# dharunm236/TempME

Hardware: AMD Instinct MI355X
Metric: explained target-edges/sec (TGN+Enron, n_degree=20) at 1/2/4/8 MI355X (higher is better)
Workload: dtype fp32

## Files before the change

include/tempme.h:

```cpp
#ifndef TEMPME_H_
#define TEMPME_H_

#include <stdint.h>

#ifdef __cplusplus
extern "C" {
#endif

#define TM_OK 0
#define TM_E_EDGE_NOT_IN_LIST (-1)
#define TM_E_SHAPE (-2)
#define TM_E_HIP (-3)
#define TM_E_ARG (-4)
#define TM_E_UNSUPPORTED (-5)

#define TM_SIDE_NONE 0
#define TM_SIDE_SRC 1
#define TM_SIDE_TGT 2
#define TM_SIDE_BGD 3
#define TM_STAGE_STEP2 16
#define TM_STAGE_STEP3 17
#define TM_STAGE_NEG 32
#define TM_STAGE_PERM 48
#define TM_SPLIT_TRAIN 0
#define TM_SPLIT_TEST 1
#define TM_SPLIT_NULL 2

typedef struct tm_graph tm_graph;
typedef struct tm_weights tm_weights;
typedef struct tm_dropin tm_dropin;

typedef struct {
    uint64_t seed;
    uint32_t split;
    uint32_t side;
} tm_rng;

const char *tm_last_error(void);
int tm_version(void);

#define TM_DEBUG_FORCE_UNKEYED 1
#define TM_DEBUG_HOST_BUILD 2
#define TM_DEBUG_GRAPH_TIMING 3
#define TM_DEBUG_WALK_BLOCKS 4
#define TM_DEBUG_N_OPTS 5
int tm_debug_set(int32_t opt, int32_t value);
int tm_set_host_threads(int32_t n);

int tm_graph_build(int32_t n_nodes, const int64_t *in_off, const int32_t *ngh, const int32_t *eid,
                   const double *ts, int device, tm_graph **out);
int tm_graph_build_edges(int32_t n_nodes, int64_t n_edges, const int64_t *src, const int64_t *dst,
                         const int64_t *eidx, const double *ts, int device, tm_graph **out);
int tm_graph_free(tm_graph *g);
int tm_graph_info(const tm_graph *g, int32_t *n_nodes, int64_t *n_entries, int32_t *max_eid);
int tm_graph_export(const tm_graph *g, int64_t *off, int32_t *ngh, int32_t *eid, double *ts, int32_t *dict_val);
int tm_graph_strict_view(const tm_graph *g, tm_graph **out);

int tm_sample_khop(const tm_graph *g, tm_rng rng, int32_t k, int32_t N, int32_t B, const int32_t *root,
                   const double *cut, const int32_t *eidx, const uint32_t *event_ids, int32_t *out_node,
                   int32_t *out_eid, float *out_ts, int32_t *err_flag, void *stream);

int tm_sample_walks(const tm_graph *g, tm_rng rng, int32_t N, int32_t M, int32_t B, const int32_t *root,
                    const int32_t *h1_node, const int32_t *h1_eid, const float *h1_ts, const uint32_t *event_ids,
                    int32_t *out_node6, int32_t *out_eid3, float *out_ts3, int32_t *out_anony3, int32_t *out_cat,
                    void *stream);

int tm_neg_sample(tm_rng rng, const int32_t *list, int64_t n_list, const uint32_t *event_ids, int32_t n, int32_t j,
                  int32_t *out, void *stream);
// ... 353 lines not shown
```

tempme_amd/_lib.py:

```python
import ctypes as C
import os
import types

import torch

_HERE = os.path.dirname(os.path.abspath(__file__))
LIB_PATH = os.environ.get("TEMPME_LIB") or os.path.join(_HERE, "lib", "libtempme_hip.so")

TM_OK = 0
TM_E_EDGE_NOT_IN_LIST = -1
TM_E_SHAPE = -2
TM_E_HIP = -3
TM_E_ARG = -4
TM_E_UNSUPPORTED = -5

SIDE_NONE, SIDE_SRC, SIDE_TGT, SIDE_BGD = 0, 1, 2, 3
SPLIT_TRAIN, SPLIT_TEST, SPLIT_NULL = 0, 1, 2
TM_DEBUG_FORCE_UNKEYED, TM_DEBUG_HOST_BUILD, TM_DEBUG_GRAPH_TIMING, TM_DEBUG_WALK_BLOCKS = 1, 2, 3, 4
N_WEIGHTS = 28

EXPORTS = (
    "tm_last_error", "tm_version", "tm_debug_set", "tm_set_host_threads", "tm_graph_build", "tm_graph_build_edges", "tm_graph_free", "tm_graph_info", "tm_graph_export",
    "tm_graph_strict_view",
    "tm_sample_khop", "tm_sample_walks", "tm_neg_sample", "tm_perm_keys", "tm_motif_hist", "tm_edge_counts",
    "tm_sample_events", "tm_gather_rows", "tm_weights_create", "tm_weights_create_ex", "tm_weights_pack", "tm_weights_variant", "tm_weights_set_node_zero", "tm_weights_version", "tm_weights_free",
    "tm_weight_split3", "tm_weight_gcn_split", "tm_encoder_workspace_bytes",
    "tm_walk_importance", "tm_encoder_pool_workspace_bytes", "tm_encoder_pool_fwd",
    "tm_encoder_pool_train_workspace_bytes", "tm_encoder_pool_train_fwd", "tm_encoder_pool_bwd", "tm_encoder_pool_wgrad",
    "tm_encoder_fwd", "tm_encoder_fwd_tab", "tm_encoder_train_supported", "tm_encoder_train_fwd", "tm_encoder_bwd", "tm_encoder_wgrad", "tm_wgrad",
    "tm_explain_train_fwd", "tm_explain_train_fwd_pad", "tm_explain_train_bwd", "tm_kl_loss", "tm_edge_importance", "tm_edge_gate_table",
    "tm_edge_table_cols", "tm_edge_tables", "tm_edge_feature_table", "tm_edge_importance_tab", "tm_tgn_attn_fwd", "tm_tgn_attn_bwd", "tm_tgn_attn_train_fwd", "tm_tgn_attn_train_bwd", "tm_tgn_attn_train_workspace_bytes", "tm_tgn_attn_train_dtab", "tm_tgn_rows_reduce", "tm_tgat_attn_fwd", "tm_tgat_attn_bwd", "tm_tgat_merge_fwd", "tm_tgat_attn_train_workspace_bytes", "tm_tgat_attn_train_fwd", "tm_tgat_attn_train_bwd", "tm_gm_packed_floats", "tm_gm_pack", "tm_gm_embed", "tm_gm_embed_bwd_ok", "tm_gm_embed_bwd", "tm_gm_packed_a_floats", "tm_gm_pack_a", "tm_gm_fused_ok", "tm_gm_train_ok", "tm_gm_train_workspace_bytes", "tm_gm_train_fwd", "tm_gm_train_bwd", "tm_dropin_create", "tm_dropin_free", "tm_dropin_forward", "tm_dropin_set_stream", "tm_dropin_gate_cache", "tm_dropin_gate_cache_clear", "tm_edge_importance_gf", "tm_edge_importance_gf3", "tm_edge_importance_gf3_bern",
    "tm_mask_least_important", "tm_profile_enable", "tm_profile_sync", "tm_profile_entry",
    "tm_beta_params", "tm_beta_rsample_bwd", "tm_adam_step", "tm_adam_step_gated", "tm_copy_many", "tm_host_register", "tm_host_unregister",
    "tm_stage_cast",
)


class TmRng(C.Structure):
    _fields_ = [("seed", C.c_uint64), ("split", C.c_uint32), ("side", C.c_uint32)]


# ... 296 lines not shown
```

tempme_amd/csrc/encoder.hip:

```cpp
#include <algorithm>
#include <atomic>
#include <cstring>
#include <vector>

#include "encoder_common.h"

namespace tmk {

__device__ __forceinline__ double block_sum(double v, double *red) {
#pragma unroll
    for (int o = 32; o > 0; o >>= 1) v += __shfl_xor(v, o);
    const int wave = threadIdx.x >> 6, nw = blockDim.x >> 6;
    __syncthreads();
    if ((threadIdx.x & 63) == 0) red[wave] = v;
    __syncthreads();
    double s = 0.0;
    for (int k = 0; k < nw; ++k) s += red[k];
    return s;
}

__global__ void __launch_bounds__(1024) std_kernel(int32_t B, int32_t W, const double *__restrict__ cut,
                                                   const float *__restrict__ ts3, float *__restrict__ std_out) {
    __shared__ double red[16];
    const int64_t g = blockIdx.x;
// ... 518 lines not shown
        o[t] = __builtin_amdgcn_mfma_f32_16x16x4f32(w.z, x[q].z, o[t], 0, 0, 0);
        p[t] = __builtin_amdgcn_mfma_f32_16x16x4f32(w.z, y[q].z, p[t], 0, 0, 0);
        o[t] = __builtin_amdgcn_mfma_f32_16x16x4f32(w.w, x[q].w, o[t], 0, 0, 0);
        p[t] = __builtin_amdgcn_mfma_f32_16x16x4f32(w.w, y[q].w, p[t], 0, 0, 0);
        __builtin_amdgcn_sched_barrier(0);
    }
}

template <int NQE>
struct WalkLay {
    static constexpr int EV = FoldLay::SIZE, EVB = EV + 11 * NQE * 256, G1 = EVB + 176, G1B = G1 + 4 * 11 * 256,
                         G2 = G1B + 64, G2B = G2 + 4 * 4 * 256, W1 = G2B + 64, W1B = W1 + 8 * 8 * 256, W2 = W1B + 128,
                         W2B = W2 + 8 * 8 * 256, A1 = W2B + 128, A1B = A1 + 4 * 8 * 256, A2 = A1B + 64,
                         A2B = A2 + 4 * 4 * 256, M1 = A2B + 64, M1B = M1 + 5 * 5 * 256, M2 = M1B + 80,
                         M2B = M2 + 4 * 5 * 256;
};

constexpr int PFP = 4;
constexpr int WALK_WAVES = 2;
constexpr int WALK_WPB = 4;

constexpr int GCN_LDS = 3;
constexpr int GCN_LDS_FRAGS = GCN_LDS * 12;
constexpr int gcn_step(int k, int gl, int ns) {
    const int nstr = ns - gl, m = nstr < gl ? nstr : gl;
    if (k < 2 * m) return (k & 1) ? k / 2 : gl + k / 2;
    return nstr > gl ? gl + k - m : k - m;
}

template <int NTO, int NQ, int NQL, int BASE>
__device__ __forceinline__ void cgemm(__amdgpu_buffer_rsrc_t wr, const floatx4 (&x)[NQ], floatx4 (&o)[NTO]) {
    using O = PairOrder<NTO, NQ>;
    const int vo = lane_id() * 16;
    constexpr int N = NTO * NQ, D = PFP < N ? PFP : N;
    auto off = [](int i) { return BASE / 4 + (O::t(i) * NQL + O::q(i)) * 64; };
    float4 buf[D];
#pragma unroll
    for (int i = 0; i < D; ++i) buf[i] = wload(wr, vo, off(i));
#pragma unroll
    for (int k = 0; k < O::NP * NQ; ++k) {
        const int i = 2 * k, t = O::t(i), q = O::q(i);
        const float4 w0 = buf[i % D];
        if (i + D < N) buf[i % D] = wload(wr, vo, off(i + D));
        const float4 w1 = buf[(i + 1) % D];
        if (i + 1 + D < N) buf[(i + 1) % D] = wload(wr, vo, off(i + 1 + D));
        o[t] = __builtin_amdgcn_mfma_f32_16x16x4f32(w0.x, x[q].x, o[t], 0, 0, 0);
// ... 154 lines not shown
__device__ __forceinline__ floatx4 relu_add4(const floatx4 &a, const float4 &b) {
    return floatx4{relu(a[0] + b.x), relu(a[1] + b.y), relu(a[2] + b.z), relu(a[3] + b.w)};
}

__device__ __forceinline__ floatx4 relu4(const floatx4 &a) {
    return floatx4{relu(a[0]), relu(a[1]), relu(a[2]), relu(a[3])};
}

struct WalkArgs {
    EncW P;
    int64_t n_slots;
    int32_t W, M, BW;
    const float *n_feat, *e_feat;
    const int32_t *node6, *eid3, *cat;
    const float *ts3, *cnt, *stdv;
    const double *cut;
    float *out;
    const float *etab;
    uint32_t *ticket;
    const float *wgt = nullptr;
};

#ifdef TM_STAMPS
__device__ unsigned long long g_st[3][10];
__device__ unsigned long long g_live;
#define TM_STAMP(k)                                 \
    do {                                            \
        __builtin_amdgcn_sched_barrier(0);          \
        T[k] = __builtin_amdgcn_s_memtime();        \
        __builtin_amdgcn_sched_barrier(0);          \
    } while (0)
#else
#define TM_STAMP(k) (void)T
#endif
#ifdef TM_TRACE
__device__ unsigned long long g_tr[8192][32];
#endif

constexpr int EQ_MAX = 4;
static_assert(EQ_MAX == 4, "load_ef holds 4 K steps");

struct PosIn {
    int32_t e, ns, nt;
    float ta, tb, c0, c1, c2;
    bool v;
    __device__ __forceinline__ int32_t edge() const { return v ? e : 0; }
};
// ... 62 lines not shown
    if constexpr (PURE) return c;
    const int k = 32 * s + 8 * g + j;
    asm volatile("" : "+v"(c));
    float v = c;
    if (k < de + 3) v = (k == de) ? c0 : (k == de + 1) ? c1 : c2;
    if (k < de) v = ETAB ? 0.f : e;
    return v;
}

__device__ __forceinline__ float4 ef_step(const float4 *erow4, int s, int hh, int g, int de) {
    const int i = 8 * s + 2 * g + hh, n4 = de >> 2;
    const float4 v = erow4[i < n4 ? i : n4 - 1];
    return i < n4 ? v : make_float4(0.f, 0.f, 0.f, 0.f);
}

#define ETAB_N(q0) ((q0) > 0 ? 11 : 1)
template <int Q0>
__device__ __forceinline__ void load_et(const WalkArgs &a, int32_t e, float4 (&et)[ETAB_N(Q0)]) {
    if constexpr (Q0 > 0) {
        const float4 *trow = reinterpret_cast<const float4 *>(a.etab + (int64_t)e * 176);
        const int g = lane_id() >> 4;
#pragma unroll
        for (int t = 0; t < 11; ++t) et[t] = trow[4 * t + g];
    }
}

template <int NQE, int NTD, bool SEF, int Q0, bool ZN, class Extra>
__device__ __forceinline__ void encode_position(const WalkArgs &a, __amdgpu_buffer_rsrc_t wr, const float *cs,
                                                const PosIn &pi, const float (&ef)[EQ_MAX][4],
                                                float4 (&et)[ETAB_N(Q0)], Extra &&extra, int p, floatx4 (&H)[8],
                                                float4 (&pre)[PFP], const NextFr &nx, unsigned long long (&T)[10],
                                                const float4 *gl) {
    constexpr bool ETAB = Q0 > 0;
    static_assert(!(ETAB && SEF), "table mode replaces the streamed edge features");
    using C = WalkConsts<NQE, NTD>;
    using LY = WalkLay<NQE>;
    const EncW &P = a.P;
    const int g = lane_id() >> 4;
    const int de = P.de, dn = P.dn;
    const float dt = pi.v ? pi.tb - pi.ta : 0.f, c0 = pi.v ? pi.c0 : 0.f, c1 = pi.v ? pi.c1 : 0.f,
                c2 = pi.v ? pi.c2 : 0.f;
    const float4 *nrow_s = reinterpret_cast<const float4 *>(a.n_feat + (int64_t)(pi.v ? pi.ns : 0) * dn);
    const float4 *nrow_t = reinterpret_cast<const float4 *>(a.n_feat + (int64_t)(pi.v ? pi.nt : 0) * dn);
    floatx4 L[NTD];
    if constexpr (ETAB) {
#pragma unroll
// ... 139 lines not shown
            if (p == 2) {
#pragma unroll
                for (int k = 0; k < D; ++k) buf[(N + k) % D] = wloadg(k);
            }
#pragma unroll
            for (int k = 0; k < D; ++k) gb[k] = buf[(N + k) % D];
        } else {
            if (p == 2) {
#pragma unroll
                for (int k = 0; k < PFP; ++k) buf[(N + k) % D] = wload(wr, vo, g1f(k));
            }
#pragma unroll
            for (int k = 0; k < PFP; ++k) pre[k] = buf[(N + k) % D];
        }
    }
    TM_STAMP(2);
    floatx4 Hs[4], Ht[4];
#pragma unroll
    for (int t = 0; t < 4; ++t) {
        Hs[t] = ldsx4(cs + C::G1, t);
        if constexpr (!ZN) Ht[t] = ldsx4(cs + C::G1C, t);
    }
    if constexpr (ZN) {
        constexpr int N = (NSG - GL) * 12, D = GD;
        static_assert(N % D == 0 && D >= PFP, "event_gcn ring depth");
        const int vo = lane_id() * 16, ln = lane_id();
        int zg = 0;
        asm volatile("" : "+s"(zg));
        auto wloadg = [&](int i) {
            return __builtin_bit_cast(float4, __builtin_amdgcn_raw_buffer_load_b128(wr, vog, zg + goff(i) * 16, 0));
        };
        auto take = [&](int i) {
            const float4 v = gb[i % D];
            if (i + D < N) gb[i % D] = wloadg(i + D);
            else if (i + D - N < PFP) gb[i % D] = wload(wr, vo, nx.o[i + D - N]);
            return v;
        };
        auto fetch = [&](int p, float4 (&w)[6]) {
            const int u = gcn_step(p / 2, GL, NSG), t = 2 * (p & 1);
#pragma unroll
            for (int k = 0; k < 6; ++k) {
                if (u < GL) w[k] = gl[((u * 4 + t) * 3 + k) * 64 + ln];
                else w[k] = take(((u - GL) * 4 + t) * 3 + k);
            }
        };
        auto act = [&](Split3 &x, int u, int j) {
            const int q = 2 * u + (j >> 2);
            if (q < NTD) {
                split_put(x, j, 0.f + relu(0.f + L[q < NTD ? q : 0][j & 3]));
            } else {
                x.h[j] = (__bf16)0.f;
                x.m[j] = (__bf16)0.f;
                x.l[j] = (__bf16)0.f;
            }
        };
        Split3 xb;
#pragma unroll
        for (int j = 0; j < 8; ++j) act(xb, gcn_step(0, GL, NSG), j);
        float4 wb[2][6];
        fetch(0, wb[0]);
#pragma unroll
        for (int k = 0; k < NSG; ++k) {
            extra(2 * k);
            if (2 * k + 1 < NTD) extra(2 * k + 1);
            Split3 xn = xb;
#pragma unroll
            for (int t = 0; t < 4; t += 2) {
                const int pp = 2 * k + t / 2;
                if (pp + 1 < 2 * NSG) fetch(pp + 1, wb[(pp + 1) & 1]);
                const float4(&w)[6] = wb[pp & 1];
                const bf16x8 h0 = __builtin_bit_cast(bf16x8, w[0]), m0 = __builtin_bit_cast(bf16x8, w[1]),
                             l0 = __builtin_bit_cast(bf16x8, w[2]), h1 = __builtin_bit_cast(bf16x8, w[3]),
                             m1 = __builtin_bit_cast(bf16x8, w[4]), l1 = __builtin_bit_cast(bf16x8, w[5]);
                Hs[t] = TM_MF32(l0, xb.h, Hs[t]);
                Hs[t + 1] = TM_MF32(l1, xb.h, Hs[t + 1]);
                Hs[t] = TM_MF32(h0, xb.l, Hs[t]);
                Hs[t + 1] = TM_MF32(h1, xb.l, Hs[t + 1]);
                Hs[t] = TM_MF32(m0, xb.m, Hs[t]);
                Hs[t + 1] = TM_MF32(m1, xb.m, Hs[t + 1]);
                Hs[t] = TM_MF32(m0, xb.h, Hs[t]);
                Hs[t + 1] = TM_MF32(m1, xb.h, Hs[t + 1]);
                Hs[t] = TM_MF32(h0, xb.m, Hs[t]);
                Hs[t + 1] = TM_MF32(h1, xb.m, Hs[t + 1]);
                Hs[t] = TM_MF32(h0, xb.h, Hs[t]);
                Hs[t + 1] = TM_MF32(h1, xb.h, Hs[t + 1]);
                if (k + 1 < NSG) {
#pragma unroll
                    for (int j = 2 * t; j < 2 * t + 4; ++j) act(xn, gcn_step(k + 1, GL, NSG), j);
                }
                __builtin_amdgcn_sched_barrier(0);
            }
            xb = xn;
        }
#pragma unroll
        for (int k = 0; k < PFP; ++k) pre[k] = gb[(N + k) % D];
    } else {
        const int vo = lane_id() * 16;
        float4 wq[2][4];
        {
#pragma unroll
            for (int q = 0; q < JN - 1 && q < NTD; ++q) nload(q);
        }
#pragma unroll
        for (int t = 0; t < 4; ++t) wq[0][t] = pre[t];
#pragma unroll
        for (int q = 0; q < NTD; ++q) {
            if (q + JN - 1 < NTD) nload(q + JN - 1);
            if (q + 1 < NTD) {
#pragma unroll
                for (int t = 0; t < 4; ++t) wq[(q + 1) & 1][t] = wload(wr, vo, LY::G1 / 4 + (t * NTD + q + 1) * 64);
            } else {
#pragma unroll
                for (int t = 0; t < 4; ++t) wq[(q + 1) & 1][t] = wload(wr, vo, nx.o[t]);
            }
            extra(q);
            const float4 xs4 = rs[q % JN], xt4 = rt[q % JN];
            const float sv[4] = {xs4.x, xs4.y, xs4.z, xs4.w}, tv[4] = {xt4.x, xt4.y, xt4.z, xt4.w};
            floatx4 A, Bq;
// ... 7 lines not shown
            for (int t = 0; t < 4; ++t) {
                const float4 w = wq[q & 1][t];
                Hs[t] = __builtin_amdgcn_mfma_f32_16x16x4f32(w.x, A.x, Hs[t], 0, 0, 0);
                Ht[t] = __builtin_amdgcn_mfma_f32_16x16x4f32(w.x, Bq.x, Ht[t], 0, 0, 0);
                Hs[t] = __builtin_amdgcn_mfma_f32_16x16x4f32(w.y, A.y, Hs[t], 0, 0, 0);
                Ht[t] = __builtin_amdgcn_mfma_f32_16x16x4f32(w.y, Bq.y, Ht[t], 0, 0, 0);
                Hs[t] = __builtin_amdgcn_mfma_f32_16x16x4f32(w.z, A.z, Hs[t], 0, 0, 0);
                Ht[t] = __builtin_amdgcn_mfma_f32_16x16x4f32(w.z, Bq.z, Ht[t], 0, 0, 0);
                Hs[t] = __builtin_amdgcn_mfma_f32_16x16x4f32(w.w, A.w, Hs[t], 0, 0, 0);
                Ht[t] = __builtin_amdgcn_mfma_f32_16x16x4f32(w.w, Bq.w, Ht[t], 0, 0, 0);
            }
            __builtin_amdgcn_sched_barrier(0);
        }
#pragma unroll
        for (int t = 0; t < 4; ++t) pre[t] = wq[NTD & 1][t];
    }
    TM_STAMP(3);
    TM_STAMP(4);
#pragma unroll
    for (int t = 0; t < 4; ++t) {
        H[t] = relu4(Hs[t]);
        H[4 + t] = ZN ? H[t] : relu4(Ht[t]);
    }
    TM_STAMP(5);
}

__device__ __forceinline__ float col_sum(float v) {
    v += __shfl_xor(v, 16);
    v += __shfl_xor(v, 32);
    return v;
}

struct HeadIn {
    double cu;
    float sd, t0, t1;
    int32_t c;
    bool v;
    float wt;
};

template <int NV>
struct Stash {
    floatx4 V[NV][64];
    floatx4 P2[4][64];
    float cw[64];
};
// ... 70 lines not shown
    }
    s0 *= tw_mult(tw0);
    s1 *= tw_mult(tw1);
    const float mx = fmaxf(s0, s1), e0 = expf(s0 - mx), e1 = expf(s1 - mx), sum = e0 + e1;
    const float al0 = e0 / sum, al1 = e1 / sum;
    floatx4 Hm[NA];
#pragma unroll
    for (int t = 0; t < NA; ++t) {
#pragma unroll
        for (int r = 0; r < 4; ++r) Hm[t][r] = al0 * H0[t][r] + al1 * H1[t][r];
    }
    floatx4 X[4];
#pragma unroll
    for (int t = 0; t < 4; ++t) X[t] = st.P2[t][lane];
    cgemm_p<4, NA, NA, ZN ? FoldLay::A1GZ : FoldLay::A1G>(wr, Hm, X, pre, nx_end);
    const float wt = (valid && hi.v) ? hi.wt : 0.f;
#pragma unroll
    for (int t = 0; t < 4; ++t) {
#pragma unroll
        for (int r = 0; r < 4; ++r) acc[t][r] = __builtin_fmaf(wt, relu(X[t][r]), acc[t][r]);
    }
}

template <bool ZN = false>
__device__ __forceinline__ float score_dot(const Stash<ZN ? 4 : 8> &st, const floatx4 (&H)[8]) {
    const int lane = threadIdx.x & 63;
    float s = 0.f;
#pragma unroll
    for (int t = 0; t < (ZN ? 4 : 8); ++t) {
        const floatx4 v = st.V[t][lane];
#pragma unroll
        for (int r = 0; r < 4; ++r) s = __builtin_fmaf(v[r], H[t][r], s);
    }
    return col_sum(s) + st.cw[lane];
}

template <int NQE, int NTD, bool SEF = false, int QE0 = 0, bool SPLIT = false, bool ZN = false, bool POOL = false>
__global__ void __launch_bounds__(64 * WALK_WPB, 4 * WALK_WAVES / WALK_WPB) walk_kernel(WalkArgs a) {
    using C = WalkConsts<NQE, NTD>;
    constexpr int NA = ZN ? 4 : 8;
    const EncW &P = a.P;
    const int lane = threadIdx.x & 63, col = lane & 15;
    const int32_t NS = a.W / a.M;
    const int64_t n_units = (a.n_slots + 15) / 16;
    constexpr bool PERSIST = !SPLIT;
    const int64_t ustride = PERSIST ? (int64_t)gridDim.x * (blockDim.x >> 6) : n_units;
    int64_t unit = (int64_t)blockIdx.x * (blockDim.x >> 6) + (threadIdx.x >> 6);
    auto ticket = [&]() -> int64_t {
        uint32_t t = 0;
        if (lane == 0) t = atomicAdd(a.ticket, 1u);
        return ustride + (int64_t)(uint32_t)__builtin_amdgcn_readfirstlane((int)t);
    };
    int m0 = 0;
    if constexpr (SPLIT) {
        m0 = (int)(unit % a.M);
        unit /= a.M;
    }
    auto coords = [&](int64_t u, bool &v, int64_t &eg_, int32_t &j_) {
        const int64_t gs = u * 16 + col;
        v = u < n_units && gs < a.n_slots;
        eg_ = v ? gs / NS : 0;
// ... 19 lines not shown
            gl[i] = P.g13[((((f / 3) % 4) * NSG + f / 12) * 3 + f % 3) * 64 + l];
        }
    }
    load_consts<NQE, NTD, ZN>(P, cs);
    __syncthreads();
#ifdef TM_TRACE
    if (lane == 0 && trw < 8192) {
        g_tr[trw][0] = tr0;
        g_tr[trw][1] = __builtin_amdgcn_s_memrealtime();
        g_tr[trw][28] = 0;
        g_tr[trw][29] = (unsigned)__builtin_amdgcn_s_getreg(63492) | ((unsigned long long)(unsigned)__builtin_amdgcn_s_getreg(30740) << 32);
    }
#endif
    if (unit >= n_units) return;
    Stash<NA> &st = stash[threadIdx.x >> 6];
    const auto wr = wrsrc(P.kv.w);
    floatx4 H0[NA];
    float s0 = 0.f;
    floatx4 PA[POOL ? 4 : 1];
    if constexpr (POOL) {
#pragma unroll
        for (int t = 0; t < 4; ++t) PA[t] = floatx4{0.f, 0.f, 0.f, 0.f};
    }
    const int n_pass = SPLIT ? 3 : 1 + 2 * a.M;
    PosIn cur = load_pos(a, eg * a.W + (int64_t)j * a.M, 2, valid);
    float ef[EQ_MAX][4] = {};
    float4 et[ETAB_N(QE0)];
    NextFr lin0;
#pragma unroll
    for (int k = 0; k < PFP; ++k) lin0.o[k] = (int)(P.ev3 - P.kv.w) + (((k / 3) * C::NS + QE0 / 2) * 3 + k % 3) * 64;
    float4 pre[PFP];
#pragma unroll
    for (int k = 0; k < PFP; ++k) pre[k] = wload(wr, lane_id() * 16, lin0.o[k]);
    if constexpr (QE0 == 0) load_ef(a, cur.edge(), ef);
    else load_et<QE0>(a, cur.edge(), et);
#ifdef TM_STAMPS
    const unsigned long long clk_t0 = __builtin_amdgcn_s_memtime(), clk_r0 = __builtin_amdgcn_s_memrealtime();
    if (lane == 0) atomicMax(&g_st[2][9], atomicAdd(&g_live, 1ull) + 1);
#endif
#pragma nounroll
    for (;;) {
    int64_t unext = unit + ustride;
    bool vn = false;
    int64_t egn = 0;
    int32_t jn = 0;
    if constexpr (!PERSIST) coords(unext, vn, egn, jn);
#pragma nounroll
    for (int pass = 0; pass < n_pass; ++pass) {
        if (PERSIST && pass + 1 == n_pass) {
            unext = ticket();
            coords(unext, vn, egn, jn);
        }
        if (PERSIST) {
            const int q = (pass * 4) / n_pass;
            if (q == 0) __builtin_amdgcn_s_setprio(3);
            else if (q == 1) __builtin_amdgcn_s_setprio(2);
            else if (q == 2) __builtin_amdgcn_s_setprio(1);
            else __builtin_amdgcn_s_setprio(0);
        }
        const int m = SPLIT ? m0 : pass == 0 ? 0 : (pass - 1) >> 1;
        const int p = pass == 0 ? 2 : ((pass - 1) & 1);
        const int64_t gw = eg * a.W + (int64_t)j * a.M + m;
        HeadIn hi{0.0, 1.f, 0.f, 0.f, -1, false};
        auto load_hi = [&]() {
            hi.v = valid;
            hi.cu = a.cut[eg];
            hi.sd = a.stdv[gw / a.BW];
            hi.t0 = a.ts3[gw * 3 + 0];
            hi.t1 = a.ts3[gw * 3 + 1];
            hi.c = a.cat[gw];
            if constexpr (POOL) hi.wt = a.wgt[gw];
        };
        const bool last = pass + 1 == n_pass;
        const int pn = !last ? ((pass & 1) == 0 ? 0 : 1) : 2;
        const int64_t gwn = !last ? eg * a.W + (int64_t)j * a.M + (SPLIT ? m0 : pass >> 1) : egn * a.W + (int64_t)jn * a.M;
        PosIn nxt;
        auto extra = [&](int q) {
            if (q == 0) {
                load_hi();
                nxt = load_pos(a, gwn, pn, !last ? valid : vn);
            }
        };
        floatx4 H[8];
        unsigned long long T[10];
        TM_STAMP(0);
        const NextFr nx_pos = ZN ? pair_first<4>(p == 2 ? FoldLay::A1DZ / 4 : FoldLay::A1GZ / 4)
                                 : pair_first<8>(p == 2 ? FoldLay::A1D / 4 : FoldLay::A1G / 4);
        encode_position<NQE, NTD, SEF, QE0, ZN>(a, wr, cs, cur, ef, et, extra, p, H, pre,
                                                p == 0 ? lin0 : nx_pos, T, gl);
        if constexpr (QE0 == 0) load_ef(a, nxt.edge(), ef);
        else load_et<QE0>(a, nxt.edge(), et);
        cur = nxt;
        TM_STAMP(6);
        floatx4 Uv[4];
#pragma unroll
        for (int t = 0; t < 4; ++t) Uv[t] = H[t];
        if (ZN && p == 2) {
            floatx4 P2[4], V[4];
#pragma unroll
            for (int t = 0; t < 4; ++t) P2[t] = ldsx4(cs + C::CP, t);
            cgemm_p<4, 4, 4, FoldLay::A1DZ>(wr, Uv, P2, pre, pair_first<4>(FoldLay::KVZ / 4));
#pragma unroll
            for (int t = 0; t < 4; ++t) V[t] = ldsx4(cs + C::V0, t);
            cgemm_p<4, 4, 4, FoldLay::KVZ>(wr, Uv, V, pre, lin0);
            TM_STAMP(7);
            float cw = 0.f;
#pragma unroll
            for (int t = 0; t < 4; ++t) {
                const float4 b = lds4(cs + C::U, t);
                cw = __builtin_fmaf(Uv[t][0], b.x, cw);
                cw = __builtin_fmaf(Uv[t][1], b.y, cw);
                cw = __builtin_fmaf(Uv[t][2], b.z, cw);
                cw = __builtin_fmaf(Uv[t][3], b.w, cw);
            }
            cw = col_sum(cw) + cs[C::C0];
// ... 37 lines not shown
#pragma unroll
            for (int t = 0; t < NA; ++t) H0[t] = H[t];
            s0 = s;
        }
        if constexpr (POOL) {
            if (p == 1) {
                if constexpr (ZN) walk_pool_head<NQE, NTD, ZN>(a, wr, valid, hi, st, s0, s, H0, Uv, pre, lin0, PA);
                else walk_pool_head<NQE, NTD, ZN>(a, wr, valid, hi, st, s0, s, H0, H, pre, lin0, PA);
                if (SPLIT || m + 1 == a.M) {
                    const int64_t row = SPLIT ? (unit * 16 + col) * a.M + m0 : unit * 16 + col;
                    float *dst = a.out + row * HID + 4 * (lane >> 4);
#pragma unroll
                    for (int t = 0; t < 4; ++t) {
                        if (valid)
                            *reinterpret_cast<float4 *>(dst + 16 * t) = make_float4(PA[t][0], PA[t][1], PA[t][2], PA[t][3]);
                        PA[t] = floatx4{0.f, 0.f, 0.f, 0.f};
                    }
                }
            }
        } else if (p == 1) {
            if constexpr (ZN) walk_head<NQE, NTD, ZN>(a, wr, cs, gw, valid, hi, st, s0, s, H0, Uv, pre, lin0);
            else walk_head<NQE, NTD, ZN>(a, wr, cs, gw, valid, hi, st, s0, s, H0, H, pre, lin0);
        }
        TM_STAMP(8);
#ifdef TM_TRACE
        if (lane == 0 && trw < 8192 && trn < 2 && pass < 7) g_tr[trw][2 + 7 * trn + pass] = __builtin_amdgcn_s_memrealtime();
#endif
#ifdef TM_STAMPS
        if (lane == 0 && blockIdx.x % 16 == 5) {
            for (int k = 0; k < 8; ++k) atomicAdd(&g_st[p][k], T[k + 1] - T[k]);
            atomicAdd(&g_st[p][8], 1ull);
        }
#endif
    }
#ifdef TM_TRACE
    if (lane == 0 && trw < 8192) {
        if (trn < 12) g_tr[trw][16 + trn] = __builtin_amdgcn_s_memrealtime();
        g_tr[trw][28] = ++trn;
    }
#endif
    unit = unext;
    if (unit >= n_units) break;
    valid = vn;
    eg = egn;
    j = jn;
    }
#ifdef TM_STAMPS
    if (lane == 0 && blockIdx.x % 16 == 5) {
        atomicAdd(&g_st[0][9], __builtin_amdgcn_s_memtime() - clk_t0);
        atomicAdd(&g_st[1][9], __builtin_amdgcn_s_memrealtime() - clk_r0);
    }
    if (lane == 0) atomicAdd(&g_live, ~0ull);
#endif
}

static bool walk_layout_ok(const EncW &P, int nqe) {
    const float *base = reinterpret_cast<const float *>(P.kv.w);
    auto at = [&](const float4 *w, int off) { return reinterpret_cast<const float *>(w) == base + off; };
    const int ev = FoldLay::SIZE, g1 = ev + 11 * nqe * 256 + 176, m2 = g1 + 4 * 11 * 256 + 64 + 4 * 4 * 256 + 64 +
                                                                     2 * (8 * 8 * 256 + 128) + 4 * 8 * 256 + 64 +
                                                                     4 * 4 * 256 + 64 + 5 * 5 * 256 + 80;
// ... 530 lines not shown
                       float *F, hipStream_t s) {
    const dim3 grid((unsigned)((n_rows + TILE_ROWS - 1) / TILE_ROWS));
    if (node_zero) gcn_kernel<true><<<grid, 256, lds, s>>>(P, n_rows, n_feat, e_feat, node6, eid3, ts3, cnt, F);
    else gcn_kernel<false><<<grid, 256, lds, s>>>(P, n_rows, n_feat, e_feat, node6, eid3, ts3, cnt, F);
}

static int head_tr(const EncW &) { return 16; }
static void launch_head(const EncW &P, int64_t n_walks, int64_t walks_per_group, int32_t W, const float *F,
                        const float *ts3, const double *cut, const int32_t *cat, const float *stdv, float *out,
                        const uint8_t *drop, float dscale, hipStream_t s) {
    const int tr = head_tr(P);
    if (tr == 32)
        head_kernel<32><<<dim3((unsigned)((n_walks + 31) / 32)), 256, head_lds(P, 32), s>>>(
            P, n_walks, walks_per_group, W, F, ts3, cut, cat, stdv, out, drop, dscale);
    else
        head_kernel<16><<<dim3((unsigned)((n_walks + 15) / 16)), 256, head_lds(P, 16), s>>>(
            P, n_walks, walks_per_group, W, F, ts3, cut, cat, stdv, out, drop, dscale);
}

constexpr int64_t WALK_SPLIT_UNITS = 512;

static bool walk_split(int64_t units, int32_t M) { return units * M <= 3 * WALK_SPLIT_UNITS && units < WALK_SPLIT_UNITS; }

template <int NQE, bool SEF = false, int Q0 = 0, bool ZN = false, bool POOL = false>
static void launch_walk(const WalkArgs &a, unsigned blocks, hipStream_t s) {
    const int64_t units = (a.n_slots + 15) / 16;
    if (walk_split(units, a.M)) {
        const unsigned sb = (unsigned)((units * a.M + WALK_WPB - 1) / WALK_WPB);
        walk_kernel<NQE, 11, SEF, Q0, true, ZN, POOL><<<dim3(sb), 64 * WALK_WPB, 0, s>>>(a);
        return;
    }
    static int cap[64] = {};
    int dev = 0;
    if (hipGetDevice(&dev) == hipSuccess && dev >= 0 && dev < 64) {
        if (cap[dev] == 0) {
            int per_cu = 0, cus = 0;
            if (hipOccupancyMaxActiveBlocksPerMultiprocessor(&per_cu, walk_kernel<NQE, 11, SEF, Q0, false, ZN, POOL>, 64 * WALK_WPB, 0) ==
                    hipSuccess &&
                hipDeviceGetAttribute(&cus, hipDeviceAttributeMultiprocessorCount, dev) == hipSuccess && per_cu > 0 &&
                cus > 0)
                cap[dev] = per_cu * cus;
            else
                cap[dev] = -1;
        }
        if (cap[dev] > 0 && blocks > (unsigned)cap[dev]) blocks = (unsigned)cap[dev];
    }
    const int dbg = debug_opt(TM_DEBUG_WALK_BLOCKS);
    if (dbg > 0 && blocks > (unsigned)dbg) blocks = (unsigned)dbg;
    walk_kernel<NQE, 11, SEF, Q0, false, ZN, POOL><<<dim3(blocks), 64 * WALK_WPB, 0, s>>>(a);
}

extern "C" int tm_encoder_fwd(const tm_weights *w, const float *n_feat, const float *e_feat, int32_t n_groups,
                              int32_t B, int32_t W, int32_t M, const int32_t *node6, const int32_t *eid3,
                              const float *ts3, const int32_t *cat, const double *cut, const float *cnt,
                              void *workspace, float *out_imp, void *stream) {
    return tm_encoder_fwd_tab(w, n_feat, e_feat, nullptr, n_groups, B, W, M, node6, eid3, ts3, cat, cut, cnt,
                              workspace, out_imp, stream);
}

static int encoder_fwd_impl(const tm_weights *w, const float *n_feat, const float *e_feat, const float *etab,
                            int32_t n_groups, int32_t B, int32_t W, int32_t M, const int32_t *node6, const int32_t *eid3,
                            const float *ts3, const int32_t *cat, const double *cut, const float *cnt, void *workspace,
                            float *out_imp, void *stream, bool do_std);

extern "C" int tm_encoder_fwd_tab(const tm_weights *w, const float *n_feat, const float *e_feat, const float *etab,
                                  int32_t n_groups, int32_t B, int32_t W, int32_t M, const int32_t *node6,
                                  const int32_t *eid3, const float *ts3, const int32_t *cat, const double *cut,
                                  const float *cnt, void *workspace, float *out_imp, void *stream) {
    return encoder_fwd_impl(w, n_feat, e_feat, etab, n_groups, B, W, M, node6, eid3, ts3, cat, cut, cnt, workspace,
                            out_imp, stream, true);
}

// ... 626 lines not shown
    if (rows == 0) return TM_OK;
    if (!gfac || !eid3 || !imp || !sub1_node || !sub1_eid || !sub2_node || !sub2_eid || !out_h1 || !out_h2)
        return fail(TM_E_ARG, "tm_edge_importance_gf: NULL pointer");
    int hbits = 6;
    while ((1 << hbits) < 2 * 3 * W) ++hbits;
    if (hbits > 14) return fail(TM_E_UNSUPPORTED, "tm_edge_importance_gf: too many walks per event");
    const size_t hlds = 2 * sizeof(int32_t) * (1u << hbits);
    hipEvent_t pe = prof_begin(S_(stream));
    explain_hash_kernel<<<dim3((unsigned)rows), 256, hlds, S_(stream)>>>(W, N, hbits, eid3, gfac, imp, sub1_node,
                                                                        sub1_eid, sub2_node, sub2_eid, out_h1, out_h2);
    TM_CHECK_LAUNCH();
    prof_end("explain_hash_kernel", S_(stream), pe);
    return TM_OK;
}

#ifdef TM_TRACE
extern "C" int tm_debug_trace(unsigned long long *host) {
    return (int)hipMemcpyFromSymbol(host, HIP_SYMBOL(tmk::g_tr), sizeof(unsigned long long) * 8192 * 32, 0,
                                    hipMemcpyDeviceToHost);
}
#endif
#ifdef TM_STAMPS
extern "C" int tm_debug_stamps(unsigned long long *host) {
    return (int)hipMemcpyFromSymbol(host, HIP_SYMBOL(tmk::g_st), sizeof(unsigned long long) * 30, 0,
                                    hipMemcpyDeviceToHost);
}
#endif
```

Measured before the change: 3.420 million.

## Encode both walk positions in one pass sharing weight loads

Adds a pair pass to the walk kernel for zero-node table mode. Each walk step now encodes the two positions together, so one streamed set of linear weights feeds MFMAs for both positions, and the GCN stage runs back to back with a ring buffer that carries over. This halves the number of passes per walk and is meant to cut repeated weight buffer loads. The cost is higher register pressure from doubled accumulators, which may lower occupancy. The old single-position path stays available through a new debug option.

After: 3.840 million, median of 6. 12.3% higher.

```diff
diff --git a/include/tempme.h b/include/tempme.h
--- a/include/tempme.h
+++ b/include/tempme.h
@@ -43,7 +43,8 @@
 #define TM_DEBUG_HOST_BUILD 2
 #define TM_DEBUG_GRAPH_TIMING 3
 #define TM_DEBUG_WALK_BLOCKS 4
-#define TM_DEBUG_N_OPTS 5
+#define TM_DEBUG_WALK_SINGLE 5
+#define TM_DEBUG_N_OPTS 6
 int tm_debug_set(int32_t opt, int32_t value);
 int tm_set_host_threads(int32_t n);
 
diff --git a/tempme_amd/_lib.py b/tempme_amd/_lib.py
--- a/tempme_amd/_lib.py
+++ b/tempme_amd/_lib.py
@@ -17,6 +17,7 @@
 SIDE_NONE, SIDE_SRC, SIDE_TGT, SIDE_BGD = 0, 1, 2, 3
 SPLIT_TRAIN, SPLIT_TEST, SPLIT_NULL = 0, 1, 2
 TM_DEBUG_FORCE_UNKEYED, TM_DEBUG_HOST_BUILD, TM_DEBUG_GRAPH_TIMING, TM_DEBUG_WALK_BLOCKS = 1, 2, 3, 4
+TM_DEBUG_WALK_SINGLE = 5
 N_WEIGHTS = 28
 
 EXPORTS = (
diff --git a/tempme_amd/csrc/encoder.hip b/tempme_amd/csrc/encoder.hip
--- a/tempme_amd/csrc/encoder.hip
+++ b/tempme_amd/csrc/encoder.hip
@@ -564,6 +564,7 @@
 
 constexpr int GCN_LDS = 3;
 constexpr int GCN_LDS_FRAGS = GCN_LDS * 12;
+constexpr int PAIR_LIN_RING = 6, PAIR_GCN_RING = 6;
 constexpr int gcn_step(int k, int gl, int ns) {
     const int nstr = ns - gl, m = nstr < gl ? nstr : gl;
     if (k < 2 * m) return (k & 1) ? k / 2 : gl + k / 2;
@@ -764,7 +765,7 @@
 };
 
 #ifdef TM_STAMPS
-__device__ unsigned long long g_st[3][10];
+__device__ unsigned long long g_st[4][10];
 __device__ unsigned long long g_live;
 #define TM_STAMP(k)                                 \
     do {                                            \
@@ -873,6 +874,88 @@
         const int g = lane_id() >> 4;
 #pragma unroll
         for (int t = 0; t < 11; ++t) et[t] = trow[4 * t + g];
+    }
+}
+
+template <int NTD, bool AGAIN, int D, class Extra>
+__device__ __forceinline__ void gcn_zn(__amdgpu_buffer_rsrc_t wr, int vog, const float4 *gl, const floatx4 (&L)[NTD],
+                                       float4 (&gb)[D], Extra &&extra, floatx4 (&Hs)[4], float4 (&pre)[PFP],
+                                       const NextFr &nx) {
+    constexpr int NSG = (NTD + 1) / 2, GL = GCN_LDS, N = (NSG - GL) * 12;
+    static_assert(N % D == 0 && D >= PFP, "event_gcn ring depth");
+    const int vo = lane_id() * 16, ln = lane_id();
+    auto goff = [](int i) { return ((((i / 3) % 4) * NSG + GL + i / 12) * 3 + i % 3) * 64; };
+    int zg = 0;
+    asm volatile("" : "+s"(zg));
+    auto wloadg = [&](int i) {
+        return __builtin_bit_cast(float4, __builtin_amdgcn_raw_buffer_load_b128(wr, vog, zg + goff(i) * 16, 0));
+    };
+    auto take = [&](int i) {
+        const float4 v = gb[i % D];
+        if (i + D < N) gb[i % D] = wloadg(i + D);
+        else if constexpr (AGAIN) gb[i % D] = wloadg(i + D - N);
+        else if (i + D - N < PFP) gb[i % D] = wload(wr, vo, nx.o[i + D - N]);
+        return v;
+    };
+    auto fetch = [&](int p, float4 (&w)[6]) {
+        const int u = gcn_step(p / 2, GL, NSG), t = 2 * (p & 1);
+#pragma unroll
+        for (int k = 0; k < 6; ++k) {
+            if (u < GL) w[k] = gl[((u * 4 + t) * 3 + k) * 64 + ln];
+            else w[k] = take(((u - GL) * 4 + t) * 3 + k);
+        }
+    };
+    auto act = [&](Split3 &x, int u, int j) {
+        const int q = 2 * u + (j >> 2);
+        if (q < NTD) {
+            split_put(x, j, 0.f + relu(0.f + L[q < NTD ? q : 0][j & 3]));
+        } else {
+            x.h[j] = (__bf16)0.f;
+            x.m[j] = (__bf16)0.f;
+            x.l[j] = (__bf16)0.f;
+        }
+    };
+    Split3 xb;
+#pragma unroll
+    for (int j = 0; j < 8; ++j) act(xb, gcn_step(0, GL, NSG), j);
+    float4 wb[2][6];
+    fetch(0, wb[0]);
+#pragma unroll
+    for (int k = 0; k < NSG; ++k) {
+        extra(2 * k);
+        if (2 * k + 1 < NTD) extra(2 * k + 1);
+        Split3 xn = xb;
+#pragma unroll
+        for (int t = 0; t < 4; t += 2) {
+            const int pp = 2 * k + t / 2;
+            if (pp + 1 < 2 * NSG) fetch(pp + 1, wb[(pp + 1) & 1]);
+            const float4(&w)[6] = wb[pp & 1];
+            const bf16x8 h0 = __builtin_bit_cast(bf16x8, w[0]), m0 = __builtin_bit_cast(bf16x8, w[1]),
+                         l0 = __builtin_bit_cast(bf16x8, w[2]), h1 = __builtin_bit_cast(bf16x8, w[3]),
+                         m1 = __builtin_bit_cast(bf16x8, w[4]), l1 = __builtin_bit_cast(bf16x8, w[5]);
+            Hs[t] = TM_MF32(l0, xb.h, Hs[t]);
+            Hs[t + 1] = TM_MF32(l1, xb.h, Hs[t + 1]);
+            Hs[t] = TM_MF32(h0, xb.l, Hs[t]);
+            Hs[t + 1] = TM_MF32(h1, xb.l, Hs[t + 1]);
+            Hs[t] = TM_MF32(m0, xb.m, Hs[t]);
+            Hs[t + 1] = TM_MF32(m1, xb.m, Hs[t + 1]);
+            Hs[t] = TM_MF32(m0, xb.h, Hs[t]);
+            Hs[t + 1] = TM_MF32(m1, xb.h, Hs[t + 1]);
+            Hs[t] = TM_MF32(h0, xb.m, Hs[t]);
+            Hs[t + 1] = TM_MF32(h1, xb.m, Hs[t + 1]);
+            Hs[t] = TM_MF32(h0, xb.h, Hs[t]);
+            Hs[t + 1] = TM_MF32(h1, xb.h, Hs[t + 1]);
+            if (k + 1 < NSG) {
+#pragma unroll
+                for (int j = 2 * t; j < 2 * t + 4; ++j) act(xn, gcn_step(k + 1, GL, NSG), j);
+            }
+            __builtin_amdgcn_sched_barrier(0);
+        }
+        xb = xn;
+    }
+    if constexpr (!AGAIN) {
+#pragma unroll
+        for (int k = 0; k < PFP; ++k) pre[k] = gb[(N + k) % D];
     }
 }
 
@@ -1058,78 +1141,7 @@
         if constexpr (!ZN) Ht[t] = ldsx4(cs + C::G1C, t);
     }
     if constexpr (ZN) {
-        constexpr int N = (NSG - GL) * 12, D = GD;
-        static_assert(N % D == 0 && D >= PFP, "event_gcn ring depth");
-        const int vo = lane_id() * 16, ln = lane_id();
-        int zg = 0;
-        asm volatile("" : "+s"(zg));
-        auto wloadg = [&](int i) {
-            return __builtin_bit_cast(float4, __builtin_amdgcn_raw_buffer_load_b128(wr, vog, zg + goff(i) * 16, 0));
-        };
-        auto take = [&](int i) {
-            const float4 v = gb[i % D];
-            if (i + D < N) gb[i % D] = wloadg(i + D);
-            else if (i + D - N < PFP) gb[i % D] = wload(wr, vo, nx.o[i + D - N]);
-            return v;
-        };
-        auto fetch = [&](int p, float4 (&w)[6]) {
-            const int u = gcn_step(p / 2, GL, NSG), t = 2 * (p & 1);
-#pragma unroll
-            for (int k = 0; k < 6; ++k) {
-                if (u < GL) w[k] = gl[((u * 4 + t) * 3 + k) * 64 + ln];
-                else w[k] = take(((u - GL) * 4 + t) * 3 + k);
-            }
-        };
-        auto act = [&](Split3 &x, int u, int j) {
-            const int q = 2 * u + (j >> 2);
-            if (q < NTD) {
-                split_put(x, j, 0.f + relu(0.f + L[q < NTD ? q : 0][j & 3]));
-            } else {
-                x.h[j] = (__bf16)0.f;
-                x.m[j] = (__bf16)0.f;
-                x.l[j] = (__bf16)0.f;
-            }
-        };
-        Split3 xb;
-#pragma unroll
-        for (int j = 0; j < 8; ++j) act(xb, gcn_step(0, GL, NSG), j);
-        float4 wb[2][6];
-        fetch(0, wb[0]);
-#pragma unroll
-        for (int k = 0; k < NSG; ++k) {
-            extra(2 * k);
-            if (2 * k + 1 < NTD) extra(2 * k + 1);
-            Split3 xn = xb;
-#pragma unroll
-            for (int t = 0; t < 4; t += 2) {
-                const int pp = 2 * k + t / 2;
-                if (pp + 1 < 2 * NSG) fetch(pp + 1, wb[(pp + 1) & 1]);
-                const float4(&w)[6] = wb[pp & 1];
-                const bf16x8 h0 = __builtin_bit_cast(bf16x8, w[0]), m0 = __builtin_bit_cast(bf16x8, w[1]),
-                             l0 = __builtin_bit_cast(bf16x8, w[2]), h1 = __builtin_bit_cast(bf16x8, w[3]),
-                             m1 = __builtin_bit_cast(bf16x8, w[4]), l1 = __builtin_bit_cast(bf16x8, w[5]);
-                Hs[t] = TM_MF32(l0, xb.h, Hs[t]);
-                Hs[t + 1] = TM_MF32(l1, xb.h, Hs[t + 1]);
-                Hs[t] = TM_MF32(h0, xb.l, Hs[t]);
-                Hs[t + 1] = TM_MF32(h1, xb.l, Hs[t + 1]);
-                Hs[t] = TM_MF32(m0, xb.m, Hs[t]);
-                Hs[t + 1] = TM_MF32(m1, xb.m, Hs[t + 1]);
-                Hs[t] = TM_MF32(m0, xb.h, Hs[t]);
-                Hs[t + 1] = TM_MF32(m1, xb.h, Hs[t + 1]);
-                Hs[t] = TM_MF32(h0, xb.m, Hs[t]);
-                Hs[t + 1] = TM_MF32(h1, xb.m, Hs[t + 1]);
-                Hs[t] = TM_MF32(h0, xb.h, Hs[t]);
-                Hs[t + 1] = TM_MF32(h1, xb.h, Hs[t + 1]);
-                if (k + 1 < NSG) {
-#pragma unroll
-                    for (int j = 2 * t; j < 2 * t + 4; ++j) act(xn, gcn_step(k + 1, GL, NSG), j);
-                }
-                __builtin_amdgcn_sched_barrier(0);
-            }
-            xb = xn;
-        }
-#pragma unroll
-        for (int k = 0; k < PFP; ++k) pre[k] = gb[(N + k) % D];
+        gcn_zn<NTD, false, GD>(wr, vog, gl, L, gb, extra, Hs, pre, nx);
     } else {
         const int vo = lane_id() * 16;
         float4 wq[2][4];
@@ -1183,6 +1195,125 @@
         H[t] = relu4(Hs[t]);
         H[4 + t] = ZN ? H[t] : relu4(Ht[t]);
     }
+    TM_STAMP(5);
+}
+
+template <int NQE, int NTD, int Q0, class Extra>
+__device__ __forceinline__ void encode_pair(const WalkArgs &a, __amdgpu_buffer_rsrc_t wr, const float *cs,
+                                            const PosIn &pi0, const PosIn &pi1, const float4 (&et0)[NTD],
+                                            const float4 (&et1)[NTD], Extra &&extra, floatx4 (&U0)[4],
+                                            floatx4 (&U1)[4], float4 (&pre)[PFP], const NextFr &nx,
+                                            unsigned long long (&T)[10], const float4 *gl) {
+    static_assert(Q0 > 0, "the pair pass starts from the edge table's rows");
+    using C = WalkConsts<NQE, NTD>;
+    const EncW &P = a.P;
+    const int g = lane_id() >> 4;
+    const int de = P.de;
+    const float dt0 = pi0.v ? pi0.tb - pi0.ta : 0.f, c00 = pi0.v ? pi0.c0 : 0.f, c01 = pi0.v ? pi0.c1 : 0.f,
+                c02 = pi0.v ? pi0.c2 : 0.f;
+    const float dt1 = pi1.v ? pi1.tb - pi1.ta : 0.f, c10 = pi1.v ? pi1.c0 : 0.f, c11 = pi1.v ? pi1.c1 : 0.f,
+                c12 = pi1.v ? pi1.c2 : 0.f;
+    floatx4 L0[NTD], L1[NTD];
+#pragma unroll
+    for (int t = 0; t < NTD; ++t) {
+        L0[t] = floatx4{et0[t].x, et0[t].y, et0[t].z, et0[t].w};
+        L1[t] = floatx4{et1[t].x, et1[t].y, et1[t].z, et1[t].w};
+    }
+    TM_STAMP(1);
+    constexpr int NSG = (NTD + 1) / 2, GL = GCN_LDS;
+    const int vog = lane_id() * 16 + 16 * (int)(P.g13 - P.kv.w);
+    constexpr int GD = PAIR_GCN_RING;
+    float4 gb[GD];
+    {
+        constexpr int NS = C::NS, S0 = Q0 / 2;
+        constexpr int N = NTD * (NS - S0) * 3, D = PAIR_LIN_RING;
+        static_assert(D >= PFP && D <= N && D % 3 == 0 && D <= GD, "lin_event ring depth");
+        const int vo3 = lane_id() * 16 + 16 * (int)(P.ev3 - P.kv.w);
+        auto off = [](int i) { return ((((i / 3) % NTD) * NS + S0 + i / (3 * NTD)) * 3 + i % 3) * 64; };
+        auto goff = [](int i) { return ((((i / 3) % 4) * NSG + GL + i / 12) * 3 + i % 3) * 64; };
+        int z3 = 0;
+        asm volatile("" : "+s"(z3));
+        auto wload3 = [&](int i) {
+            return __builtin_bit_cast(float4, __builtin_amdgcn_raw_buffer_load_b128(wr, vo3, z3 + off(i) * 16, 0));
+        };
+        auto wloadg = [&](int i) {
+            return __builtin_bit_cast(float4, __builtin_amdgcn_raw_buffer_load_b128(wr, vog, z3 + goff(i) * 16, 0));
+        };
+        float4 buf[D];
+#pragma unroll
+        for (int i = 0; i < D; ++i) buf[i] = i < PFP ? pre[i] : wload3(i);
+        auto pure = [](int s) { return s > S0; };
+        const float *cw = cs + C::XW, *cp = cs + C::XP;
+        Split3 xs0, xs1;
+        {
+            float w8[8], p8[8];
+            lds8(cw, S0, w8);
+            lds8(cp, S0, p8);
+#pragma unroll
+            for (int j = 0; j < 8; ++j) {
+                split_put(xs0, j, gen_one<true, false>(S0, j, w8[j], p8[j], 0.f, g, de, dt0, c00, c01, c02));
+                split_put(xs1, j, gen_one<true, false>(S0, j, w8[j], p8[j], 0.f, g, de, dt1, c10, c11, c12));
+            }
+        }
+#pragma unroll
+        for (int s = S0; s < NS; ++s) {
+            Split3 xn0 = xs0, xn1 = xs1;
+            auto gen = [&](int j) {
+                if (s + 1 < NS && j < 8) {
+                    const float w = cw[32 * (s + 1) + 8 * g + j], ph = cp[32 * (s + 1) + 8 * g + j];
+                    const float v0 = pure(s + 1) ? gen_one<true, true>(s + 1, j, w, ph, 0.f, g, de, dt0, c00, c01, c02)
+                                                 : gen_one<true, false>(s + 1, j, w, ph, 0.f, g, de, dt0, c00, c01, c02);
+                    const float v1 = pure(s + 1) ? gen_one<true, true>(s + 1, j, w, ph, 0.f, g, de, dt1, c10, c11, c12)
+                                                 : gen_one<true, false>(s + 1, j, w, ph, 0.f, g, de, dt1, c10, c11, c12);
+                    split_put(xn0, j, v0);
+                    split_put(xn1, j, v1);
+                }
+            };
+            auto take = [&](int i) {
+                const bf16x8 v = __builtin_bit_cast(bf16x8, buf[i % D]);
+                if (i + D < N) buf[i % D] = wload3(i + D);
+                else buf[i % D] = wloadg(i + D - N);
+                return v;
+            };
+#pragma unroll
+            for (int t = 0; t < NTD; ++t) {
+                const int i = ((s - S0) * NTD + t) * 3;
+                const bf16x8 h = take(i), m = take(i + 1), l = take(i + 2);
+                L0[t] = TM_MF32(l, xs0.h, L0[t]);
+                L1[t] = TM_MF32(l, xs1.h, L1[t]);
+                L0[t] = TM_MF32(h, xs0.l, L0[t]);
+                L1[t] = TM_MF32(h, xs1.l, L1[t]);
+                L0[t] = TM_MF32(m, xs0.m, L0[t]);
+                L1[t] = TM_MF32(m, xs1.m, L1[t]);
+                L0[t] = TM_MF32(m, xs0.h, L0[t]);
+                L1[t] = TM_MF32(m, xs1.h, L1[t]);
+                L0[t] = TM_MF32(h, xs0.m, L0[t]);
+                L1[t] = TM_MF32(h, xs1.m, L1[t]);
+                L0[t] = TM_MF32(h, xs0.h, L0[t]);
+                L1[t] = TM_MF32(h, xs1.h, L1[t]);
+                gen(t);
+                __builtin_amdgcn_sched_barrier(0);
+            }
+            xs0 = xn0;
+            xs1 = xn1;
+        }
+#pragma unroll
+        for (int k = 0; k < GD; ++k) gb[k] = k < D ? buf[(N + k) % D] : wloadg(k);
+    }
+    TM_STAMP(2);
+    floatx4 Hs[4];
+#pragma unroll
+    for (int t = 0; t < 4; ++t) Hs[t] = ldsx4(cs + C::G1, t);
+    gcn_zn<NTD, true, GD>(wr, vog, gl, L0, gb, [](int) {}, Hs, pre, nx);
+#pragma unroll
+    for (int t = 0; t < 4; ++t) U0[t] = relu4(Hs[t]);
+    TM_STAMP(3);
+#pragma unroll
+    for (int t = 0; t < 4; ++t) Hs[t] = ldsx4(cs + C::G1, t);
+    gcn_zn<NTD, false, GD>(wr, vog, gl, L1, gb, extra, Hs, pre, nx);
+    TM_STAMP(4);
+#pragma unroll
+    for (int t = 0; t < 4; ++t) U1[t] = relu4(Hs[t]);
     TM_STAMP(5);
 }
 
@@ -1299,8 +1430,9 @@
     }
 }
 
-template <bool ZN = false>
-__device__ __forceinline__ float score_dot(const Stash<ZN ? 4 : 8> &st, const floatx4 (&H)[8]) {
+template <bool ZN = false, int NH>
+__device__ __forceinline__ float score_dot(const Stash<ZN ? 4 : 8> &st, const floatx4 (&H)[NH]) {
+    static_assert(NH >= (ZN ? 4 : 8), "a position's hidden vector");
     const int lane = threadIdx.x & 63;
     float s = 0.f;
 #pragma unroll
@@ -1312,8 +1444,10 @@
     return col_sum(s) + st.cw[lane];
 }
 
-template <int NQE, int NTD, bool SEF = false, int QE0 = 0, bool SPLIT = false, bool ZN = false, bool POOL = false>
+template <int NQE, int NTD, bool SEF = false, int QE0 = 0, bool SPLIT = false, bool ZN = false, bool POOL = false,
+          bool PAIR = false>
 __global__ void __launch_bounds__(64 * WALK_WPB, 4 * WALK_WAVES / WALK_WPB) walk_kernel(WalkArgs a) {
+    static_assert(!PAIR || (ZN && QE0 > 0 && !SEF && !POOL), "the pair pass: zero-node table mode, not pooled");
     using C = WalkConsts<NQE, NTD>;
     constexpr int NA = ZN ? 4 : 8;
     const EncW &P = a.P;
@@ -1379,10 +1513,13 @@
 #pragma unroll
         for (int t = 0; t < 4; ++t) PA[t] = floatx4{0.f, 0.f, 0.f, 0.f};
     }
-    const int n_pass = SPLIT ? 3 : 1 + 2 * a.M;
+    const int n_pass = PAIR ? (SPLIT ? 2 : 1 + a.M) : (SPLIT ? 3 : 1 + 2 * a.M);
     PosIn cur = load_pos(a, eg * a.W + (int64_t)j * a.M, 2, valid);
+    PosIn cur1 = cur;
     float ef[EQ_MAX][4] = {};
     float4 et[ETAB_N(QE0)];
+    float4 et1[PAIR ? ETAB_N(QE0) : 1];
+    (void)cur1, (void)et1;
     NextFr lin0;
 #pragma unroll
     for (int k = 0; k < PFP; ++k) lin0.o[k] = (int)(P.ev3 - P.kv.w) + (((k / 3) * C::NS + QE0 / 2) * 3 + k % 3) * 64;
@@ -1402,8 +1539,7 @@
     int64_t egn = 0;
     int32_t jn = 0;
     if constexpr (!PERSIST) coords(unext, vn, egn, jn);
-#pragma nounroll
-    for (int pass = 0; pass < n_pass; ++pass) {
+    auto run_pass = [&](const int pass, const int pt) __attribute__((always_inline)) {
         if (PERSIST && pass + 1 == n_pass) {
             unext = ticket();
             coords(unext, vn, egn, jn);
@@ -1415,8 +1551,7 @@
             else if (q == 2) __builtin_amdgcn_s_setprio(1);
             else __builtin_amdgcn_s_setprio(0);
         }
-        const int m = SPLIT ? m0 : pass == 0 ? 0 : (pass - 1) >> 1;
-        const int p = pass == 0 ? 2 : ((pass - 1) & 1);
+        const int m = SPLIT ? m0 : pass == 0 ? 0 : PAIR ? pass - 1 : (pass - 1) >> 1;
         const int64_t gw = eg * a.W + (int64_t)j * a.M + m;
         HeadIn hi{0.0, 1.f, 0.f, 0.f, -1, false};
         auto load_hi = [&]() {
@@ -1429,18 +1564,36 @@
             if constexpr (POOL) hi.wt = a.wgt[gw];
         };
         const bool last = pass + 1 == n_pass;
-        const int pn = !last ? ((pass & 1) == 0 ? 0 : 1) : 2;
-        const int64_t gwn = !last ? eg * a.W + (int64_t)j * a.M + (SPLIT ? m0 : pass >> 1) : egn * a.W + (int64_t)jn * a.M;
-        PosIn nxt;
+        const int pn = !last ? (PAIR || (pass & 1) == 0 ? 0 : 1) : 2;
+        const int64_t gwn = !last ? eg * a.W + (int64_t)j * a.M + (SPLIT ? m0 : PAIR ? pass : pass >> 1)
+                                  : egn * a.W + (int64_t)jn * a.M;
+        PosIn nxt, nxt1;
         auto extra = [&](int q) {
             if (q == 0) {
                 load_hi();
                 nxt = load_pos(a, gwn, pn, !last ? valid : vn);
+                if constexpr (PAIR) nxt1 = load_pos(a, gwn, 1, !last ? valid : vn);
             }
         };
-        floatx4 H[8];
         unsigned long long T[10];
         TM_STAMP(0);
+        if (PAIR && pt == 3) {
+            if constexpr (PAIR) {
+                floatx4 U0[4], U1[4];
+                encode_pair<NQE, NTD, QE0>(a, wr, cs, cur, cur1, et, et1, extra, U0, U1, pre,
+                                           pair_first<4>(FoldLay::A1GZ / 4), T, gl);
+                load_et<QE0>(a, nxt.edge(), et);
+                load_et<QE0>(a, nxt1.edge(), et1);
+                cur = nxt;
+                cur1 = nxt1;
+                TM_STAMP(6);
+                const float sc0 = score_dot<true>(st, U0), sc1 = score_dot<true>(st, U1);
+                TM_STAMP(7);
+                walk_head<NQE, NTD, true>(a, wr, cs, gw, valid, hi, st, sc0, sc1, U0, U1, pre, lin0);
+            }
+        } else {
+        const int p = PAIR ? 2 : pt;
+        floatx4 H[8];
         const NextFr nx_pos = ZN ? pair_first<4>(p == 2 ? FoldLay::A1DZ / 4 : FoldLay::A1GZ / 4)
                                  : pair_first<8>(p == 2 ? FoldLay::A1D / 4 : FoldLay::A1G / 4);
         encode_position<NQE, NTD, SEF, QE0, ZN>(a, wr, cs, cur, ef, et, extra, p, H, pre,
@@ -1448,6 +1601,10 @@
         if constexpr (QE0 == 0) load_ef(a, nxt.edge(), ef);
         else load_et<QE0>(a, nxt.edge(), et);
         cur = nxt;
+        if constexpr (PAIR) {
+            load_et<QE0>(a, nxt1.edge(), et1);
+            cur1 = nxt1;
+        }
         TM_STAMP(6);
         floatx4 Uv[4];
 #pragma unroll
@@ -1531,21 +1688,31 @@
             if constexpr (ZN) walk_head<NQE, NTD, ZN>(a, wr, cs, gw, valid, hi, st, s0, s, H0, Uv, pre, lin0);
             else walk_head<NQE, NTD, ZN>(a, wr, cs, gw, valid, hi, st, s0, s, H0, H, pre, lin0);
         }
+        }
         TM_STAMP(8);
 #ifdef TM_TRACE
         if (lane == 0 && trw < 8192 && trn < 2 && pass < 7) g_tr[trw][2 + 7 * trn + pass] = __builtin_amdgcn_s_memrealtime();
 #endif
 #ifdef TM_STAMPS
         if (lane == 0 && blockIdx.x % 16 == 5) {
-            for (int k = 0; k < 8; ++k) atomicAdd(&g_st[p][k], T[k + 1] - T[k]);
-            atomicAdd(&g_st[p][8], 1ull);
+            for (int k = 0; k < 8; ++k) atomicAdd(&g_st[pt][k], T[k + 1] - T[k]);
+            atomicAdd(&g_st[pt][8], 1ull);
         }
 #endif
+    };
+    if constexpr (PAIR) {
+        run_pass(0, 2);
+#pragma nounroll
+        for (int pass = 1; pass < n_pass; ++pass) run_pass(pass, 3);
+    } else {
+#pragma nounroll
+        for (int pass = 0; pass < n_pass; ++pass) run_pass(pass, pass == 0 ? 2 : ((pass - 1) & 1));
     }
 #ifdef TM_TRACE
     if (lane == 0 && trw < 8192) {
         if (trn < 12) g_tr[trw][16 + trn] = __builtin_amdgcn_s_memrealtime();
         g_tr[trw][28] = ++trn;
+        g_tr[trw][30] = (unsigned long long)n_pass;
     }
 #endif
     unit = unext;
@@ -2122,12 +2289,12 @@
 
 static bool walk_split(int64_t units, int32_t M) { return units * M <= 3 * WALK_SPLIT_UNITS && units < WALK_SPLIT_UNITS; }
 
-template <int NQE, bool SEF = false, int Q0 = 0, bool ZN = false, bool POOL = false>
-static void launch_walk(const WalkArgs &a, unsigned blocks, hipStream_t s) {
+template <int NQE, bool SEF, int Q0, bool ZN, bool POOL, bool PAIR>
+static void launch_walk_as(const WalkArgs &a, unsigned blocks, hipStream_t s) {
     const int64_t units = (a.n_slots + 15) / 16;
     if (walk_split(units, a.M)) {
         const unsigned sb = (unsigned)((units * a.M + WALK_WPB - 1) / WALK_WPB);
-        walk_kernel<NQE, 11, SEF, Q0, true, ZN, POOL><<<dim3(sb), 64 * WALK_WPB, 0, s>>>(a);
+        walk_kernel<NQE, 11, SEF, Q0, true, ZN, POOL, PAIR><<<dim3(sb), 64 * WALK_WPB, 0, s>>>(a);
         return;
     }
     static int cap[64] = {};
@@ -2135,7 +2302,7 @@
     if (hipGetDevice(&dev) == hipSuccess && dev >= 0 && dev < 64) {
         if (cap[dev] == 0) {
             int per_cu = 0, cus = 0;
-            if (hipOccupancyMaxActiveBlocksPerMultiprocessor(&per_cu, walk_kernel<NQE, 11, SEF, Q0, false, ZN, POOL>, 64 * WALK_WPB, 0) ==
+            if (hipOccupancyMaxActiveBlocksPerMultiprocessor(&per_cu, walk_kernel<NQE, 11, SEF, Q0, false, ZN, POOL, PAIR>, 64 * WALK_WPB, 0) ==
                     hipSuccess &&
                 hipDeviceGetAttribute(&cus, hipDeviceAttributeMultiprocessorCount, dev) == hipSuccess && per_cu > 0 &&
                 cus > 0)
@@ -2147,7 +2314,15 @@
     }
     const int dbg = debug_opt(TM_DEBUG_WALK_BLOCKS);
     if (dbg > 0 && blocks > (unsigned)dbg) blocks = (unsigned)dbg;
-    walk_kernel<NQE, 11, SEF, Q0, false, ZN, POOL><<<dim3(blocks), 64 * WALK_WPB, 0, s>>>(a);
+    walk_kernel<NQE, 11, SEF, Q0, false, ZN, POOL, PAIR><<<dim3(blocks), 64 * WALK_WPB, 0, s>>>(a);
+}
+
+template <int NQE, bool SEF = false, int Q0 = 0, bool ZN = false, bool POOL = false>
+static void launch_walk(const WalkArgs &a, unsigned blocks, hipStream_t s) {
+    if constexpr (ZN && Q0 > 0 && !SEF && !POOL) {
+        if (!debug_opt(TM_DEBUG_WALK_SINGLE)) return launch_walk_as<NQE, SEF, Q0, ZN, POOL, true>(a, blocks, s);
+    }
+    launch_walk_as<NQE, SEF, Q0, ZN, POOL, false>(a, blocks, s);
 }
 
 extern "C" int tm_encoder_fwd(const tm_weights *w, const float *n_feat, const float *e_feat, int32_t n_groups,
@@ -2820,7 +2995,7 @@
 #endif
 #ifdef TM_STAMPS
 extern "C" int tm_debug_stamps(unsigned long long *host) {
-    return (int)hipMemcpyFromSymbol(host, HIP_SYMBOL(tmk::g_st), sizeof(unsigned long long) * 30, 0,
+    return (int)hipMemcpyFromSymbol(host, HIP_SYMBOL(tmk::g_st), sizeof(unsigned long long) * 40, 0,
                                     hipMemcpyDeviceToHost);
 }
 #endif
```
